# guanjq/targetdiff

Measured on NVIDIA H100. Metric: molecules/sec (1000-step sampling, CrossDocked pocket shape), higher is better.
Workload: dtype f32 (storage, LayerNorm, softmax, accumulation); GEMM operands as 2-piece bf16 splits on wgmma (3 products, ~16-bit operand mantissa)

## Files before the change

targetdiff_b200/csrc/edge_mlp_v4.cu:

```cuda
#include <stdio.h>
#include <stdlib.h>
#include <string.h>

#include "tdiff_common.cuh"
#include "hopper_mma.cuh"

namespace v4 {

constexpr int kTile = 64;
constexpr int kTabClassBytes = 2 * 128 * 128;
constexpr int kSrcStride = 512 + 32, kDst = 8;
constexpr int sSrc = 0, sDstRows = sSrc + kTile * kSrcStride, sMeta = sDstRows + kDst * 512, kStage = sMeta + kTile * 16;
constexpr int kMAtom = 32 * 128, kMPiece = 2 * kMAtom, kMImg = 2 * kMPiece;
template <int NOUT, bool FOLD>
struct Map {
  static constexpr int kCons = (NOUT == 128 && !FOLD) ? 3 : 2;
  static constexpr int kThreads = (kCons + 1) * 128;
  static constexpr int kProdRegs = kCons == 3 ? 32 : 40, kConsRegs = kCons == 3 ? 160 : 232;
  static constexpr int W = 0, T = W + 4 * 128 * 128, Par = T + kTabClassBytes, X = Par + 2 * 128 * 4,
                       M = X + kCons * 4 * 2 * 128 * 4, C = M + (FOLD ? kCons * kMImg : 0), Stage = C + (FOLD ? kCons * 32 * 4 : 0),
                       Bar = Stage + kCons * kStage, Smem = Bar + 8 * (1 + 2 * kCons);
  static constexpr bool kOrdered = kCons == 2;
  static constexpr int kPairBar = 1, kOrderBar = kPairBar + 2 * kCons, kFoldBar = kOrderBar + kCons;
  static_assert(M % 1024 == 0 && Stage % 128 == 0 && kStage % 128 == 0 && Smem <= 227 * 1024, "shared-memory map");
  static_assert(128 * kProdRegs + kCons * 128 * kConsRegs == kThreads * (65536 / kThreads / 8 * 8), "register split");
  static_assert(kFoldBar + kCons <= 16, "named barriers");
};

__device__ __forceinline__ uint32_t smem_u32(const void* p) { return (uint32_t)__cvta_generic_to_shared(p); }
__device__ __forceinline__ void mbar_init(uint32_t bar, uint32_t count) {
  asm volatile("mbarrier.init.shared::cta.b64 [%0], %1;" ::"r"(bar), "r"(count) : "memory");
}
__device__ __forceinline__ void mbar_wait(uint32_t bar, uint32_t parity) {
  asm volatile(
      "{\n\t.reg .pred p;\n\tWAIT_LOOP:\n\tmbarrier.try_wait.parity.shared::cta.b64 p, [%0], %1;\n\t@p bra WAIT_DONE;\n\tbra WAIT_LOOP;\n\t"
      "WAIT_DONE:\n\t}" ::"r"(bar), "r"(parity) : "memory");
}
__device__ __forceinline__ void mbar_expect_tx(uint32_t bar, uint32_t bytes) {
  asm volatile("mbarrier.arrive.expect_tx.shared::cta.b64 _, [%0], %1;" ::"r"(bar), "r"(bytes) : "memory");
}
__device__ __forceinline__ void bulk_g2s(uint32_t smem_dst, const void* gsrc, uint32_t bytes, uint32_t bar) {
  asm volatile("cp.async.bulk.shared::cluster.global.mbarrier::complete_tx::bytes [%0], [%1], %2, [%3];" ::"r"(smem_dst), "l"(gsrc), "r"(bytes),
               "r"(bar) : "memory");
}
__device__ __forceinline__ void fence_barrier_init() { asm volatile("fence.mbarrier_init.release.cluster;" ::: "memory"); }
__device__ __forceinline__ void mbar_arrive(uint32_t bar) { asm volatile("mbarrier.arrive.shared::cta.b64 _, [%0];" ::"r"(bar) : "memory"); }
__device__ __forceinline__ void mbar_expect_tx_only(uint32_t bar, uint32_t bytes) {
  asm volatile("mbarrier.expect_tx.shared::cta.b64 [%0], %1;" ::"r"(bar), "r"(bytes) : "memory");
}
__device__ __forceinline__ void named_bar_sync(int id, int nthreads) { asm volatile("bar.sync %0, %1;" ::"r"(id), "r"(nthreads) : "memory"); }
__device__ __forceinline__ void named_bar_arrive(int id, int nthreads) { asm volatile("bar.arrive %0, %1;" ::"r"(id), "r"(nthreads) : "memory"); }
template <int N> __device__ __forceinline__ void setmaxnreg_inc() { asm volatile("setmaxnreg.inc.sync.aligned.u32 %0;" ::"n"(N)); }
template <int N> __device__ __forceinline__ void setmaxnreg_dec() { asm volatile("setmaxnreg.dec.sync.aligned.u32 %0;" ::"n"(N)); }

__device__ __forceinline__ uint32_t cvt_bf16x2(float hi, float lo) {
  uint32_t d;
  asm("cvt.rn.bf16x2.f32 %0, %1, %2;" : "=r"(d) : "f"(hi), "f"(lo));
  return d;
}
__device__ __forceinline__ float ex2_approx(float x) { float y; asm("ex2.approx.ftz.f32 %0, %1;" : "=f"(y) : "f"(x)); return y; }
__device__ __forceinline__ void stg64(float* p, float a, float b) { asm volatile("st.global.v2.f32 [%0], {%1,%2};" ::"l"(p), "f"(a), "f"(b) : "memory"); }
__device__ __forceinline__ void stg128(float* p, float a, float b, float c, float d) {
  asm volatile("st.global.v4.f32 [%0], {%1,%2,%3,%4};" ::"l"(p), "f"(a), "f"(b), "f"(c), "f"(d) : "memory");
}

struct LnParams { float b[128]; float b2[128]; float mu[20]; };
struct AggArgs {
  const float* logits;
  const float* e_w;
  float* h;
  int key_softmax;
};

template <int N, int M, int LO_BIT>
__device__ __forceinline__ void transpose_reduce(float (&t)[N], int lane) {
  if constexpr (N > M) {
    constexpr int h = (N / M / 2) << LO_BIT;
    const bool up = lane & h;
#pragma unroll
    for (int i = 0; i < N / 2; ++i) {
      const float send = up ? t[i] : t[i + N / 2];
      const float keep = up ? t[i + N / 2] : t[i];
      t[i] = keep + __shfl_xor_sync(0xffffffffu, send, h);
    }
    transpose_reduce<N / 2, M, LO_BIT>(reinterpret_cast<float(&)[N / 2]>(t), lane);
  }
}
__device__ __forceinline__ void split2(float y0, float y1, uint32_t& hi, uint32_t& lo) {
  hi = cvt_bf16x2(y1, y0);
  const float r0 = __fsub_rn(y0, __uint_as_float(hi << 16)), r1 = __fsub_rn(y1, __uint_as_float(hi & 0xffff0000u));
  lo = cvt_bf16x2(r1, r0);
}

}

using namespace v4;

template <int NOUT, bool FOLD>
__global__ void __launch_bounds__(Map<NOUT, FOLD>::kThreads, 1)
edge_mlp_v4_kernel(const float* __restrict__ P, int zero_row, const int* __restrict__ src, const unsigned char* __restrict__ etype,
                   const float* __restrict__ dist_arr, const int* __restrict__ row_nodes, long long n_dst, long long split_dst,
                   const int* __restrict__ d_counts, int k, int offA, int offB, const unsigned char* __restrict__ w2_image,
                   const unsigned char* __restrict__ tab_image, float coeff, const float* __restrict__ qnode, float* __restrict__ out, int out_by_slot, AggArgs agg,
                   int cls, const __grid_constant__ LnParams lp) {
  static_assert(!FOLD || NOUT == 128, "the fold applies to the key MLPs");
  using L = Map<NOUT, FOLD>;
  constexpr int kCons = L::kCons, kThreads = L::kThreads;
  extern __shared__ __align__(1024) unsigned char smem_raw[];
  const uint32_t sbase = smem_u32(smem_raw);
  const uint32_t sW = sbase + L::W, sT = sbase + L::T, sBar = sbase + L::Bar;
  float* const s_b = reinterpret_cast<float*>(smem_raw + L::Par);
  float* const s_b2 = s_b + 128;
  const int tid = threadIdx.x, lane = tid & 31, warp = __shfl_sync(0xffffffffu, tid >> 5, 0);
  const int w = warp & 3, q = lane & 3;
  const int kshift = (k & (k - 1)) == 0 ? __ffs(k) - 1 : -1;
  auto row_dst = [&](long long idx, int& j) -> unsigned {
    const unsigned a = kshift >= 0 ? (unsigned)idx >> kshift : (unsigned)idx / (unsigned)k;
    j = (int)((unsigned)idx - a * (unsigned)k);
    return a;
  };

  if ((sbase & 1023u) != 0) __trap();
  if (d_counts) { n_dst = d_counts[0]; split_dst = d_counts[1]; }
  const long long n_rows = n_dst * k, split_rows = split_dst * k;
  const long long row_lo = cls ? split_rows : 0, row_hi = cls ? n_rows : split_rows;
  const long long n_tiles = row_hi > row_lo ? (row_hi - row_lo + kTile - 1) / kTile : 0;
  const long long my_tiles = (n_tiles > blockIdx.x) ? (n_tiles - blockIdx.x + gridDim.x - 1) / gridDim.x : 0;
  auto full_bar = [&](int c) { return sBar + 8u * (1 + c); };
  auto empty_bar = [&](int c) { return sBar + 8u * (1 + kCons + c); };

  constexpr int kWAtom = NOUT * 128;
  constexpr int kWPiece = 2 * kWAtom;
  constexpr uint32_t kWBytes = FOLD ? 4u * 128 * 128 : 2u * kWPiece;
  if (tid == 0) {
    mbar_init(sBar, 1);
    for (int c = 0; c < kCons; ++c) { mbar_init(full_bar(c), 32); mbar_init(empty_bar(c), 128); }
    fence_barrier_init();
    mbar_expect_tx(sBar, kWBytes + kTabClassBytes);
    bulk_g2s(sW, w2_image, kWBytes, sBar);
    bulk_g2s(sT, tab_image + (size_t)cls * kTabClassBytes, kTabClassBytes, sBar);
  }
  for (int i = tid; i < 128; i += kThreads) { s_b[i] = lp.b[i]; s_b2[i] = lp.b2[i]; }
  __syncthreads();

  if (warp < 4) {
    setmaxnreg_dec<L::kProdRegs>();
    if (warp >= kCons) return;
    const int c = warp;
    const uint32_t st = sbase + L::Stage + (uint32_t)c * kStage;
    for (long long it = c, use = 0; it < my_tiles; it += kCons, ++use) {
      const long long tile = blockIdx.x + it * (long long)gridDim.x, row0 = row_lo + tile * kTile;
      int j0;
      const unsigned a0 = row_dst(row0, j0);
      const long long last = (row0 + kTile - 1 < row_hi ? row0 + kTile - 1 : row_hi - 1);
      const int n_d = min(kDst, (int)(row_dst(last, j0) - a0) + 1);
      int s[2];
      int4 meta[2];
#pragma unroll
      for (int h = 0; h < 2; ++h) {
        const long long idx = row0 + lane + 32 * h;
        int jj = 0, ty = 3, slot = 0, node = -1;
        float dist = 0.f;
        s[h] = -1;
        if (idx < n_rows) {
          const unsigned a = row_dst(idx, jj);
          slot = a - a0 < (unsigned)kDst ? (int)(a - a0) + 1 : 0;
          node = row_nodes[a];
          if (node >= 0) {
            const size_t e = (size_t)node * k + jj;
            s[h] = src[e]; ty = etype[e]; dist = dist_arr[e];
          }
        }
        meta[h] = make_int4(node, s[h], __float_as_int(dist), ty | (slot << 8) | (jj << 16));
      }
      int dnode = -1;
      if (lane < n_d) dnode = row_nodes[a0 + lane];
      mbar_wait(empty_bar(c), (uint32_t)(use & 1) ^ 1u);
#pragma unroll
      for (int h = 0; h < 2; ++h) *reinterpret_cast<int4*>(smem_raw + L::Stage + c * kStage + sMeta + 16 * (lane + 32 * h)) = meta[h];
      if (lane == 0) mbar_expect_tx_only(full_bar(c), (uint32_t)(kTile + (FOLD ? 2 : 1) * n_d) * 512u);
      __syncwarp();
#pragma unroll
      for (int h = 0; h < 2; ++h)
        bulk_g2s(st + sSrc + (uint32_t)(lane + 32 * h) * kSrcStride, P + (size_t)(s[h] >= 0 ? s[h] : zero_row) * TD_NPROJ + offB, 512u, full_bar(c));
      if (lane < n_d) bulk_g2s(st + sDstRows + (uint32_t)lane * 512u, P + (size_t)(dnode >= 0 ? dnode : zero_row) * TD_NPROJ + offA, 512u, full_bar(c));
      if (FOLD && lane < n_d) bulk_g2s(st + sDstRows + (uint32_t)(2 + lane) * 512u, qnode + (size_t)(dnode >= 0 ? dnode : 0) * TD_H, 512u, full_bar(c));
      mbar_arrive(full_bar(c));
    }
    return;
  }

  setmaxnreg_inc<L::kConsRegs>();
  const int cwg = (warp >> 2) - 1;
  float mu[5];
#pragma unroll
  for (int m = 0; m < 5; ++m) mu[m] = lp.mu[5 * q + m];
  const float coeff2 = coeff * 1.4426950408889634f;
  mbar_wait(sBar, 0);

  const int r_base = 16 * w + (lane >> 2);
  const int pair_bar = L::kPairBar + 2 * cwg + (w >> 1);
  float* const xslot = reinterpret_cast<float*>(smem_raw + L::X) + (size_t)(cwg * 4 + w) * 256;
  float* const xpart = xslot + ((w & 1) ? -256 : 256);
  const bool do_agg = !FOLD && NOUT == 128 && qnode == nullptr && agg.logits != nullptr;
  const bool key_sm = NOUT == 128 && qnode != nullptr && agg.key_softmax;
  const unsigned char* const stage = smem_raw + L::Stage + cwg * kStage;
  const int ct = tid & 127, fu = ct & 7, fg = ct >> 3;
  const int fhd = 8 * (fg & 1) + 4 * (fu >> 2) + (fu & 3), fs = fu >> 2, frun = (fg >> 1) ^ (((fu >> 1) & 1) << 2);
  const int fn0 = 16 * ((fhd >> 1) & 1) + 2 * (fhd >> 2) + (fhd & 1);
  unsigned char* const mimg = smem_raw + L::M + cwg * kMImg;
  float* const s_c = reinterpret_cast<float*>(smem_raw + L::C) + cwg * 32;
  const int srow = k == 32 ? (w >> 1) : 0;
  const int order_mine = L::kOrderBar + cwg, order_next = L::kOrderBar + (cwg + 1) % kCons;
  auto order_wait = [&] { if constexpr (L::kOrdered) named_bar_sync(order_mine, 256); };
  auto order_pass = [&] { if constexpr (L::kOrdered) named_bar_arrive(order_next, 256); };
  const long long n_iter = (my_tiles + kCons - 1) / kCons;
  if (n_iter == 0) return;
  if (cwg == kCons - 1) order_pass();
  int set = 0;

  for (long long n = 0; n < n_iter; ++n, set ^= 1) {
    const long long it = n * kCons + cwg;
    if (it >= my_tiles) {
      if constexpr (L::kOrdered)
        for (int phase = 0; phase < 2; ++phase) { order_wait(); order_pass(); }
      continue;
    }
    const long long row0 = row_lo + (blockIdx.x + it * (long long)gridDim.x) * kTile;
    long long idx[2];
    int node[2], s[2], ty[2], jj[2], dsl[2];
    float dist[2];
    mbar_wait(full_bar(cwg), (uint32_t)(n & 1));
#pragma unroll
    for (int h = 0; h < 2; ++h) {
      idx[h] = row0 + r_base + 8 * h;
      const int4 m4 = *reinterpret_cast<const int4*>(stage + sMeta + 16 * (r_base + 8 * h));
      node[h] = m4.x; s[h] = m4.y; dist[h] = __int_as_float(m4.z);
      ty[h] = m4.w & 0xff; dsl[h] = ((m4.w >> 8) & 0xff) - 1; jj[h] = m4.w >> 16;
    }
    float ewp[2] = {0.f, 0.f};
    float4 qf[2][2];
    if constexpr (FOLD) {
#pragma unroll
      for (int h = 0; h < 2; ++h)
        if (key_sm && idx[h] < n_rows && node[h] >= 0) ewp[h] = agg.e_w[(size_t)node[h] * k + jj[h]];
#pragma unroll
      for (int sl = 0; sl < 2; ++sl)
#pragma unroll
        for (int hf = 0; hf < 2; ++hf) {
          float4 v = make_float4(0.f, 0.f, 0.f, 0.f);
          if (sl == 0 || k == 32) {
            v = *reinterpret_cast<const float4*>(stage + sDstRows + (2 + sl) * 512 + 32 * fhd + 16 * (hf ^ fs));
            v.x *= 0.35355339059327373f; v.y *= 0.35355339059327373f; v.z *= 0.35355339059327373f; v.w *= 0.35355339059327373f;
          }
          qf[sl][hf] = v;
        }
    }
    uint32_t ghi[4][4], glo[4][4];
#pragma unroll
    for (int h = 0; h < 2; ++h) {
      const bool ok = s[h] >= 0;
      float v[8];
#pragma unroll
      for (int m = 0; m < 5; ++m) {
        const float t = dist[h] - mu[m];
        v[m] = ok ? ex2_approx(coeff2 * (t * t)) : 0.0f;
      }
      v[5] = (ok && q == 3) ? 1.0f : 0.0f;
      v[6] = v[7] = 0.0f;
      const int half = ty[h] < 2 ? 1 : 0;
#pragma unroll
      for (int kk = 0; kk < 4; ++kk)
#pragma unroll
        for (int hk = 0; hk < 2; ++hk) {
          uint32_t hi, lo;
          split2(v[4 * (kk & 1) + 2 * hk], v[4 * (kk & 1) + 2 * hk + 1], hi, lo);
          const bool own = (kk >> 1) == half;
          ghi[kk][h + 2 * hk] = own ? hi : 0u;
          glo[kk][h + 2 * hk] = own ? lo : 0u;
        }
    }
    float x[64];
#pragma unroll
    for (int h = 0; h < 2; ++h) {
      const bool valid = s[h] >= 0;
      const float* ps = reinterpret_cast<const float*>(stage + sSrc + (r_base + 8 * h) * kSrcStride) + 2 * q;
      const float* pd = (dsl[h] >= 0 ? reinterpret_cast<const float*>(stage + sDstRows + dsl[h] * 512)
                                     : P + (size_t)(valid ? node[h] : zero_row) * TD_NPROJ + offA) + 2 * q;
#pragma unroll
      for (int i = 0; i < 16; ++i) {
        const float2 b = *reinterpret_cast<const float2*>(ps + 8 * i);
        float2 a = make_float2(0.f, 0.f);
        if (valid) a = *reinterpret_cast<const float2*>(pd + 8 * i);
        x[4 * i + 2 * h] = __fadd_rn(b.x, a.x);
        x[4 * i + 2 * h + 1] = __fadd_rn(b.y, a.y);
      }
    }
    mbar_arrive(empty_bar(cwg));
    wgmma_fence();
    order_wait();
#pragma unroll
    for (int term = 0; term < 3; ++term) {
#pragma unroll
      for (int kk = 0; kk < 4; ++kk)
        wgmma_n128_rs(x, term == 2 ? glo[kk] : ghi[kk], gmma_desc_sw128(sT + (term == 1 ? kTabClassBytes / 2 : 0) + kk * 32),
                      1u);
    }
    wgmma_commit();
    order_pass();
    if constexpr (FOLD) {
      const float* const w2s = reinterpret_cast<const float*>(smem_raw + L::W) + 8 * fhd;
#pragma unroll
      for (int jr = 0; jr < 2; ++jr) {
        const int f0 = 64 * jr + 8 * frun;
        float mv[2][8];
#pragma unroll
        for (int jf = 0; jf < 8; ++jf) {
          const float4 wa = *reinterpret_cast<const float4*>(w2s + (f0 + jf) * 128 + 4 * fs);
          const float4 wb = *reinterpret_cast<const float4*>(w2s + (f0 + jf) * 128 + 4 * (fs ^ 1));
#pragma unroll
          for (int sl = 0; sl < 2; ++sl) {
            const float4 qa = qf[sl][0], qb = qf[sl][1];
            const float pa = __fmaf_rn(wa.w, qa.w, __fmaf_rn(wa.z, qa.z, __fmaf_rn(wa.y, qa.y, wa.x * qa.x)));
            const float pb = __fmaf_rn(wb.w, qb.w, __fmaf_rn(wb.z, qb.z, __fmaf_rn(wb.y, qb.y, wb.x * qb.x)));
            mv[sl][jf] = pa + pb;
          }
        }
#pragma unroll
        for (int sl = 0; sl < 2; ++sl) {
          uint4 hi, lo;
          split2(mv[sl][0], mv[sl][1], hi.x, lo.x);
          split2(mv[sl][2], mv[sl][3], hi.y, lo.y);
          split2(mv[sl][4], mv[sl][5], hi.z, lo.z);
          split2(mv[sl][6], mv[sl][7], hi.w, lo.w);
          const int nr = fn0 + 8 * sl;
          const int off = jr * kMAtom + (nr >> 3) * 1024 + (nr & 7) * 128 + ((frun ^ (nr & 7)) << 4);
          *reinterpret_cast<uint4*>(mimg + off) = hi;
          *reinterpret_cast<uint4*>(mimg + kMPiece + off) = lo;
        }
      }
      if (fg < 2)
#pragma unroll
        for (int sl = 0; sl < 2; ++sl) {
          const float4 ba = *reinterpret_cast<const float4*>(s_b2 + 8 * fhd + 4 * fs), bb = *reinterpret_cast<const float4*>(s_b2 + 8 * fhd + 4 * (fs ^ 1));
          const float4 qa = qf[sl][0], qb = qf[sl][1];
          const float pa = __fmaf_rn(ba.w, qa.w, __fmaf_rn(ba.z, qa.z, __fmaf_rn(ba.y, qa.y, ba.x * qa.x)));
          const float pb = __fmaf_rn(bb.w, qb.w, __fmaf_rn(bb.z, qb.z, __fmaf_rn(bb.y, qb.y, bb.x * qb.x)));
          s_c[16 * sl + fhd] = pa + pb;
        }
      asm volatile("fence.proxy.async.shared::cta;" ::: "memory");
    }
    wgmma_wait_all();
    float rstd[2];
#pragma unroll
    for (int h = 0; h < 2; ++h) {
      float qa = 0.f, qb = 0.f;
#pragma unroll
      for (int i = 0; i < 16; ++i) {
        qa = __fmaf_rn(x[4 * i + 2 * h], x[4 * i + 2 * h], qa);
        qb = __fmaf_rn(x[4 * i + 2 * h + 1], x[4 * i + 2 * h + 1], qb);
      }
      float var = qa + qb;
      var += __shfl_xor_sync(0xffffffffu, var, 1);
      var += __shfl_xor_sync(0xffffffffu, var, 2);
      rstd[h] = rsqrtf(var * (1.0f / 128.0f) + 1e-5f);
    }
    uint32_t ahi[8][4], alo[8][4];
#pragma unroll
    for (int kk = 0; kk < 8; ++kk)
#pragma unroll
      for (int r = 0; r < 4; ++r) {
        const int h = r & 1, col = 16 * kk + 8 * (r >> 1) + 2 * q, e = 8 * kk + 2 * r;
        const float2 b = *reinterpret_cast<const float2*>(s_b + col);
        const float y0 = __fmaf_rn(x[e], rstd[h], b.x), y1 = __fmaf_rn(x[e + 1], rstd[h], b.y);
        split2(fmaxf(y0, 0.f), fmaxf(y1, 0.f), ahi[kk][r], alo[kk][r]);
      }
    float o[NOUT / 2];
    if constexpr (FOLD) {
      named_bar_sync(L::kFoldBar + cwg, 128);
#pragma unroll
      for (int sl = 0; sl < 2; ++sl) {
        const float4 cv = *reinterpret_cast<const float4*>(s_c + 16 * sl + 4 * q);
#pragma unroll
        for (int h = 0; h < 2; ++h) {
          o[4 * sl + 2 * h] = cv.x; o[4 * sl + 2 * h + 1] = cv.y;
          o[4 * (2 + sl) + 2 * h] = cv.z; o[4 * (2 + sl) + 2 * h + 1] = cv.w;
        }
      }
    }
    wgmma_fence();
    order_wait();
#pragma unroll
    for (int term = 0; term < 3; ++term) {
#pragma unroll
      for (int kk = 0; kk < 8; ++kk) {
        if constexpr (FOLD) {
          const uint64_t desc = gmma_desc_sw128(sbase + L::M + cwg * kMImg + (term == 1 ? kMPiece : 0) + (kk >> 2) * kMAtom + (kk & 3) * 32);
          wgmma_n32_rs(reinterpret_cast<float(&)[16]>(o), term == 2 ? alo[kk] : ahi[kk], desc, 1u);
        } else {
          const uint64_t desc = gmma_desc_sw128(sW + (term == 1 ? kWPiece : 0) + (kk >> 2) * kWAtom + (kk & 3) * 32);
          if constexpr (NOUT == 128) wgmma_n128_rs(o, term == 2 ? alo[kk] : ahi[kk], desc, (term | kk) ? 1u : 0u);
          else wgmma_n16_rs(o, term == 2 ? alo[kk] : ahi[kk], desc, (term | kk) ? 1u : 0u);
        }
      }
    }
    wgmma_commit();
    order_pass();
    wgmma_wait_all();

    long long orow[2];
    bool owrite[2];
#pragma unroll
    for (int h = 0; h < 2; ++h) {
      orow[h] = out_by_slot ? ((long long)node[h] * k + jj[h]) : idx[h];
      owrite[h] = idx[h] < n_rows && node[h] >= 0;
    }
    if constexpr (NOUT == 16) {
#pragma unroll
      for (int h = 0; h < 2; ++h)
        if (owrite[h])
#pragma unroll
          for (int i = 0; i < 2; ++i) {
            const float2 bb = *reinterpret_cast<const float2*>(s_b2 + 8 * i + 2 * q);
            stg64(out + (size_t)orow[h] * 16 + 8 * i + 2 * q, o[4 * i + 2 * h] + bb.x, o[4 * i + 2 * h + 1] + bb.y);
          }
    } else if (do_agg) {
      const int dnode = node[0];
      const bool active = dnode >= 0;
      const int ccol = 64 * (w & 1) + 2 * lane;
      float2 hin = make_float2(0.f, 0.f);
      if (active) hin = *reinterpret_cast<const float2*>(agg.h + (size_t)dnode * TD_H + ccol);
      float wt[2][16];
#pragma unroll
      for (int h = 0; h < 2; ++h)
#pragma unroll
        for (int i = 0; i < 4; ++i) {
          float4 t4 = make_float4(0.f, 0.f, 0.f, 0.f);
          if (active) t4 = __ldg(reinterpret_cast<const float4*>(agg.logits + (size_t)idx[h] * TD_HEADS + 4 * i));
          wt[h][4 * i] = t4.x; wt[h][4 * i + 1] = t4.y; wt[h][4 * i + 2] = t4.z; wt[h][4 * i + 3] = t4.w;
        }
      float t[32];
#pragma unroll
      for (int i = 0; i < 16; ++i) {
        const float2 bb = *reinterpret_cast<const float2*>(s_b2 + 8 * i + 2 * q);
#pragma unroll
        for (int c = 0; c < 2; ++c) {
          const float b = c ? bb.y : bb.x;
          t[2 * i + c] = __fadd_rn(__fmul_rn(__fadd_rn(o[4 * i + c], b), wt[0][i]), __fmul_rn(__fadd_rn(o[4 * i + 2 + c], b), wt[1][i]));
        }
      }
      transpose_reduce<32, 4, 2>(t, lane);
      float* slot = xslot + 128 * set;
      const int c0 = 16 * (lane >> 2) + 2 * q;
      *reinterpret_cast<float2*>(slot + c0) = make_float2(t[0], t[1]);
      *reinterpret_cast<float2*>(slot + c0 + 8) = make_float2(t[2], t[3]);
      named_bar_sync(pair_bar, 64);
      if (active) {
        const float* se = ((w & 1) ? xpart : xslot) + 128 * set;
        const float* so = ((w & 1) ? xslot : xpart) + 128 * set;
        const float2 a = *reinterpret_cast<const float2*>(se + ccol), b = *reinterpret_cast<const float2*>(so + ccol);
        *reinterpret_cast<float2*>(agg.h + (size_t)dnode * TD_H + ccol) = make_float2(hin.x + (a.x + b.x), hin.y + (a.y + b.y));
      }
    } else if (!FOLD && qnode == nullptr) {
#pragma unroll
      for (int h = 0; h < 2; ++h)
        if (owrite[h])
#pragma unroll
          for (int i = 0; i < 16; ++i) {
            const float2 bb = *reinterpret_cast<const float2*>(s_b2 + 8 * i + 2 * q);
            stg64(out + (size_t)orow[h] * 128 + 8 * i + 2 * q, o[4 * i + 2 * h] + bb.x, o[4 * i + 2 * h + 1] + bb.y);
          }
    } else {
      float lg[32];
      if constexpr (FOLD) {
#pragma unroll
        for (int h = 0; h < 2; ++h)
#pragma unroll
          for (int u = 0; u < 4; ++u) {
            const int e0 = 4 * (2 * (u >> 1)) + 2 * h + (u & 1);
            lg[4 * h + u] = srow ? o[e0 + 4] : o[e0];
          }
      } else {
#pragma unroll
        for (int h = 0; h < 2; ++h) {
          const float* qrow = qnode + (size_t)(node[h] >= 0 ? node[h] : 0) * TD_H + 2 * q;
#pragma unroll
          for (int i = 0; i < 16; ++i) {
            const float2 qv = __ldg(reinterpret_cast<const float2*>(qrow + 8 * i));
            const float2 bb = *reinterpret_cast<const float2*>(s_b2 + 8 * i + 2 * q);
            lg[8 * (i >> 2) + 4 * h + (i & 3)] = __fmaf_rn(o[4 * i + 2 * h + 1] + bb.y, qv.y, (o[4 * i + 2 * h] + bb.x) * qv.x);
          }
        }
        transpose_reduce<32, 8, 0>(lg, lane);
#pragma unroll
        for (int u = 0; u < 8; ++u) lg[u] *= 0.35355339059327373f;
      }
      if (key_sm) {
        bool valid_e[2];
        float ew[2];
#pragma unroll
        for (int h = 0; h < 2; ++h) {
          valid_e[h] = false; ew[h] = 0.f;
          if (owrite[h]) {
            valid_e[h] = s[h] >= 0;
            ew[h] = FOLD ? ewp[h] : agg.e_w[(size_t)node[h] * k + jj[h]];
          }
        }
        float mx[4], sm[4];
#pragma unroll
        for (int u = 0; u < 4; ++u) {
          lg[u] = valid_e[0] ? lg[u] * 1.4426950408889634f : -INFINITY;
          lg[4 + u] = valid_e[1] ? lg[4 + u] * 1.4426950408889634f : -INFINITY;
          mx[u] = fmaxf(lg[u], lg[4 + u]);
#pragma unroll
          for (int m = 4; m < 32; m <<= 1) mx[u] = fmaxf(mx[u], __shfl_xor_sync(0xffffffffu, mx[u], m));
        }
        if (lane < 4) *reinterpret_cast<float4*>(xslot + 4 * q) = make_float4(mx[0], mx[1], mx[2], mx[3]);
        named_bar_sync(pair_bar, 64);
        const float4 pm = *reinterpret_cast<const float4*>(xpart + 4 * q);
        mx[0] = fmaxf(mx[0], pm.x); mx[1] = fmaxf(mx[1], pm.y); mx[2] = fmaxf(mx[2], pm.z); mx[3] = fmaxf(mx[3], pm.w);
#pragma unroll
        for (int u = 0; u < 4; ++u) {
          lg[u] = valid_e[0] ? ex2_approx(lg[u] - mx[u]) : 0.0f;
          lg[4 + u] = valid_e[1] ? ex2_approx(lg[4 + u] - mx[u]) : 0.0f;
          sm[u] = lg[u] + lg[4 + u];
#pragma unroll
          for (int m = 4; m < 32; m <<= 1) sm[u] += __shfl_xor_sync(0xffffffffu, sm[u], m);
        }
        if (lane < 4) *reinterpret_cast<float4*>(xslot + 128 + 4 * q) = make_float4(sm[0], sm[1], sm[2], sm[3]);
        named_bar_sync(pair_bar, 64);
        const float4 ps = *reinterpret_cast<const float4*>(xpart + 128 + 4 * q);
        const float pl[4] = {ps.x, ps.y, ps.z, ps.w};
#pragma unroll
        for (int u = 0; u < 4; ++u) {
          const float l = sm[u] + pl[u];
          const float inv = l > 0.0f ? 1.0f / l : 0.0f;
          lg[u] = lg[u] * ew[0] * inv;
          lg[4 + u] = lg[4 + u] * ew[1] * inv;
        }
#pragma unroll
        for (int h = 0; h < 2; ++h)
          if (idx[h] < n_rows) stg128(out + (size_t)idx[h] * TD_HEADS + 4 * q, lg[4 * h], lg[4 * h + 1], lg[4 * h + 2], lg[4 * h + 3]);
      } else {
#pragma unroll
        for (int h = 0; h < 2; ++h)
          if (owrite[h]) stg128(out + (size_t)orow[h] * TD_HEADS + 4 * q, lg[4 * h], lg[4 * h + 1], lg[4 * h + 2], lg[4 * h + 3]);
      }
    }
  }
  if (cwg == 0) order_wait();
}

void td_launch_edge_mlp_v4(const float* P, int zero_row, const int* src, const unsigned char* etype, const float* dist, const int* row_nodes, long long n_dst,
                           long long split_dst, const int* d_counts, int k, const TdMlp& m, const float* h_offsets, float coeff,
                           const float* h_ln_b, const float* h_b2, const float* qnode, float* out, int out_by_slot,
                           const float* agg_logits, const float* agg_e_w, float* agg_h, int key_softmax, int sm_count, cudaStream_t st) {
  if (n_dst == 0) return;
  LnParams lp;
  memcpy(lp.b, h_ln_b, sizeof(lp.b));
  memset(lp.b2, 0, sizeof(lp.b2));
  memcpy(lp.b2, h_b2, sizeof(float) * (size_t)m.nout);
  memcpy(lp.mu, h_offsets, sizeof(lp.mu));
  static size_t opted128[TD_MAX_DEVICES] = {0}, opted16[TD_MAX_DEVICES] = {0}, optedF[TD_MAX_DEVICES] = {0};
  td_opt_in_smem(edge_mlp_v4_kernel<128, false>, Map<128, false>::Smem, opted128);
  td_opt_in_smem(edge_mlp_v4_kernel<16, false>, Map<16, false>::Smem, opted16);
  td_opt_in_smem(edge_mlp_v4_kernel<128, true>, Map<128, true>::Smem, optedF);
  AggArgs agg = {agg_logits, agg_e_w, agg_h, (key_softmax && k == 32) ? 1 : 0};
  const bool fold = m.nout == 128 && qnode && (k == 32 || k == 64);
  const long long n_cls[2] = {split_dst, n_dst - split_dst};
  for (int cls = 0; cls < 2; ++cls) {
    if (n_cls[cls] == 0) continue;
    const long long n_tiles = (n_cls[cls] * k + kTile - 1) / kTile;
    const int grid = (int)(n_tiles < sm_count ? n_tiles : sm_count);
    if (m.nout == 16)
      edge_mlp_v4_kernel<16, false><<<grid, Map<16, false>::kThreads, Map<16, false>::Smem, st>>>(
          P, zero_row, src, etype, dist, row_nodes, n_dst, split_dst, d_counts, k, m.offA, m.offB, m.w2_img, m.tabcls_img, coeff, nullptr,
          out, out_by_slot, agg, cls, lp);
    else if (fold)
      edge_mlp_v4_kernel<128, true><<<grid, Map<128, true>::kThreads, Map<128, true>::Smem, st>>>(
          P, zero_row, src, etype, dist, row_nodes, n_dst, split_dst, d_counts, k, m.offA, m.offB,
          reinterpret_cast<const unsigned char*>(m.w2t), m.tabcls_img, coeff, qnode, out, out_by_slot, agg, cls, lp);
    else
      edge_mlp_v4_kernel<128, false><<<grid, Map<128, false>::kThreads, Map<128, false>::Smem, st>>>(
          P, zero_row, src, etype, dist, row_nodes, n_dst, split_dst, d_counts, k, m.offA, m.offB, m.w2_img, m.tabcls_img, coeff, qnode,
          out, out_by_slot, agg, cls, lp);
  }
}
```

Measured before the change: 19.02.

## Replace key-MLP fold with TMA-staged query/h rows in a double-buffered epilogue area

Removes the FOLD variant, which precomputed W2·q images per tile on CUDA cores and ran a narrow N=32 wgmma. Key MLPs now use the plain 3-consumer N=128 path. The producer warp bulk-copies each destination node's query row (or h row for the value/aggregation role) and the edge weights into a double-buffered epilogue region guarded by new mbarriers, so epilogues read from shared memory instead of global. The trade-off is a full N=128 second GEMM for keys plus the qdot and transpose reduction, in exchange for removing the fold arithmetic and getting 3 consumers instead of 2.

```diff
diff --git a/targetdiff_b200/csrc/edge_mlp_v4.cu b/targetdiff_b200/csrc/edge_mlp_v4.cu
--- a/targetdiff_b200/csrc/edge_mlp_v4.cu
+++ b/targetdiff_b200/csrc/edge_mlp_v4.cu
@@ -1,6 +1,8 @@
 #include <stdio.h>
 #include <stdlib.h>
 #include <string.h>
+
+#include <type_traits>
 
 #include "tdiff_common.cuh"
 #include "hopper_mma.cuh"
@@ -11,20 +13,27 @@
 constexpr int kTabClassBytes = 2 * 128 * 128;
 constexpr int kSrcStride = 512 + 32, kDst = 8;
 constexpr int sSrc = 0, sDstRows = sSrc + kTile * kSrcStride, sMeta = sDstRows + kDst * 512, kStage = sMeta + kTile * 16;
-constexpr int kMAtom = 32 * 128, kMPiece = 2 * kMAtom, kMImg = 2 * kMPiece;
-template <int NOUT, bool FOLD>
+constexpr int sEpi = sDstRows + 2 * 512, kEpiHalf = 3 * 512, sEpiEw = 2 * 512;
+static_assert(sEpi + 2 * kEpiHalf == sMeta && sEpiEw + kTile * 4 <= kEpiHalf, "epilogue area");
+
+struct RoleKey {};
+struct RoleValue {};
+struct RolePlain {};
+
+template <int NOUT, class R>
 struct Map {
-  static constexpr int kCons = (NOUT == 128 && !FOLD) ? 3 : 2;
+  static constexpr bool kKey = std::is_same<R, RoleKey>::value, kValue = std::is_same<R, RoleValue>::value;
+  static_assert(NOUT == 128 || !(kKey || kValue), "the key and fused-aggregation epilogues need NOUT = 128");
+  static constexpr int kCons = NOUT == 128 ? 3 : 2;
   static constexpr int kThreads = (kCons + 1) * 128;
   static constexpr int kProdRegs = kCons == 3 ? 32 : 40, kConsRegs = kCons == 3 ? 160 : 232;
   static constexpr int W = 0, T = W + 4 * 128 * 128, Par = T + kTabClassBytes, X = Par + 2 * 128 * 4,
-                       M = X + kCons * 4 * 2 * 128 * 4, C = M + (FOLD ? kCons * kMImg : 0), Stage = C + (FOLD ? kCons * 32 * 4 : 0),
-                       Bar = Stage + kCons * kStage, Smem = Bar + 8 * (1 + 2 * kCons);
+                       Stage = X + kCons * 4 * 2 * 128 * 4, Bar = Stage + kCons * kStage, Smem = Bar + 8 * (1 + 4 * kCons);
   static constexpr bool kOrdered = kCons == 2;
-  static constexpr int kPairBar = 1, kOrderBar = kPairBar + 2 * kCons, kFoldBar = kOrderBar + kCons;
-  static_assert(M % 1024 == 0 && Stage % 128 == 0 && kStage % 128 == 0 && Smem <= 227 * 1024, "shared-memory map");
+  static constexpr int kPairBar = 1, kOrderBar = kPairBar + 2 * kCons;
+  static_assert(T % 1024 == 0 && Stage % 128 == 0 && kStage % 128 == 0 && Smem <= 227 * 1024, "shared-memory map");
   static_assert(128 * kProdRegs + kCons * 128 * kConsRegs == kThreads * (65536 / kThreads / 8 * 8), "register split");
-  static_assert(kFoldBar + kCons <= 16, "named barriers");
+  static_assert(kOrderBar + kCons <= 16, "named barriers");
 };
 
 __device__ __forceinline__ uint32_t smem_u32(const void* p) { return (uint32_t)__cvta_generic_to_shared(p); }
@@ -96,16 +105,16 @@
 
 using namespace v4;
 
-template <int NOUT, bool FOLD>
-__global__ void __launch_bounds__(Map<NOUT, FOLD>::kThreads, 1)
+template <int NOUT, class R>
+__global__ void __launch_bounds__(Map<NOUT, R>::kThreads, 1)
 edge_mlp_v4_kernel(const float* __restrict__ P, int zero_row, const int* __restrict__ src, const unsigned char* __restrict__ etype,
                    const float* __restrict__ dist_arr, const int* __restrict__ row_nodes, long long n_dst, long long split_dst,
                    const int* __restrict__ d_counts, int k, int offA, int offB, const unsigned char* __restrict__ w2_image,
                    const unsigned char* __restrict__ tab_image, float coeff, const float* __restrict__ qnode, float* __restrict__ out, int out_by_slot, AggArgs agg,
                    int cls, const __grid_constant__ LnParams lp) {
-  static_assert(!FOLD || NOUT == 128, "the fold applies to the key MLPs");
-  using L = Map<NOUT, FOLD>;
+  using L = Map<NOUT, R>;
   constexpr int kCons = L::kCons, kThreads = L::kThreads;
+  constexpr bool kKey = L::kKey, kValue = L::kValue;
   extern __shared__ __align__(1024) unsigned char smem_raw[];
   const uint32_t sbase = smem_u32(smem_raw);
   const uint32_t sW = sbase + L::W, sT = sbase + L::T, sBar = sbase + L::Bar;
@@ -126,15 +135,20 @@
   const long long row_lo = cls ? split_rows : 0, row_hi = cls ? n_rows : split_rows;
   const long long n_tiles = row_hi > row_lo ? (row_hi - row_lo + kTile - 1) / kTile : 0;
   const long long my_tiles = (n_tiles > blockIdx.x) ? (n_tiles - blockIdx.x + gridDim.x - 1) / gridDim.x : 0;
+  const bool epi = (kKey || kValue) && (k == 32 || k == 64);
+  const bool key_sm = kKey && agg.key_softmax && k == 32;
   auto full_bar = [&](int c) { return sBar + 8u * (1 + c); };
   auto empty_bar = [&](int c) { return sBar + 8u * (1 + kCons + c); };
+  auto epi_bar = [&](int c, int hf) { return sBar + 8u * (1 + 2 * kCons + 2 * c + hf); };
 
   constexpr int kWAtom = NOUT * 128;
   constexpr int kWPiece = 2 * kWAtom;
-  constexpr uint32_t kWBytes = FOLD ? 4u * 128 * 128 : 2u * kWPiece;
+  constexpr uint32_t kWBytes = 2u * kWPiece;
   if (tid == 0) {
     mbar_init(sBar, 1);
-    for (int c = 0; c < kCons; ++c) { mbar_init(full_bar(c), 32); mbar_init(empty_bar(c), 128); }
+    for (int c = 0; c < kCons; ++c) {
+      mbar_init(full_bar(c), 32); mbar_init(empty_bar(c), 128); mbar_init(epi_bar(c, 0), 128); mbar_init(epi_bar(c, 1), 128);
+    }
     fence_barrier_init();
     mbar_expect_tx(sBar, kWBytes + kTabClassBytes);
     bulk_g2s(sW, w2_image, kWBytes, sBar);
@@ -156,12 +170,14 @@
       const int n_d = min(kDst, (int)(row_dst(last, j0) - a0) + 1);
       int s[2];
       int4 meta[2];
+      float ew[2];
 #pragma unroll
       for (int h = 0; h < 2; ++h) {
         const long long idx = row0 + lane + 32 * h;
         int jj = 0, ty = 3, slot = 0, node = -1;
         float dist = 0.f;
         s[h] = -1;
+        ew[h] = 0.f;
         if (idx < n_rows) {
           const unsigned a = row_dst(idx, jj);
           slot = a - a0 < (unsigned)kDst ? (int)(a - a0) + 1 : 0;
@@ -169,22 +185,30 @@
           if (node >= 0) {
             const size_t e = (size_t)node * k + jj;
             s[h] = src[e]; ty = etype[e]; dist = dist_arr[e];
+            if (key_sm) ew[h] = agg.e_w[e];
           }
         }
         meta[h] = make_int4(node, s[h], __float_as_int(dist), ty | (slot << 8) | (jj << 16));
       }
       int dnode = -1;
       if (lane < n_d) dnode = row_nodes[a0 + lane];
+      const bool erow = epi && lane < n_d && dnode >= 0;
+      const int n_erow = __popc(__ballot_sync(0xffffffffu, erow));
+      const int ea = sEpi + (int)(use & 1) * kEpiHalf;
       mbar_wait(empty_bar(c), (uint32_t)(use & 1) ^ 1u);
-#pragma unroll
-      for (int h = 0; h < 2; ++h) *reinterpret_cast<int4*>(smem_raw + L::Stage + c * kStage + sMeta + 16 * (lane + 32 * h)) = meta[h];
-      if (lane == 0) mbar_expect_tx_only(full_bar(c), (uint32_t)(kTile + (FOLD ? 2 : 1) * n_d) * 512u);
+      if (epi) mbar_wait(epi_bar(c, (int)(use & 1)), (uint32_t)((use >> 1) & 1) ^ 1u);
+#pragma unroll
+      for (int h = 0; h < 2; ++h) {
+        *reinterpret_cast<int4*>(smem_raw + L::Stage + c * kStage + sMeta + 16 * (lane + 32 * h)) = meta[h];
+        if (key_sm) *reinterpret_cast<float*>(smem_raw + L::Stage + c * kStage + ea + sEpiEw + 4 * (lane + 32 * h)) = ew[h];
+      }
+      if (lane == 0) mbar_expect_tx_only(full_bar(c), (uint32_t)(kTile + n_d + n_erow) * 512u);
       __syncwarp();
 #pragma unroll
       for (int h = 0; h < 2; ++h)
         bulk_g2s(st + sSrc + (uint32_t)(lane + 32 * h) * kSrcStride, P + (size_t)(s[h] >= 0 ? s[h] : zero_row) * TD_NPROJ + offB, 512u, full_bar(c));
       if (lane < n_d) bulk_g2s(st + sDstRows + (uint32_t)lane * 512u, P + (size_t)(dnode >= 0 ? dnode : zero_row) * TD_NPROJ + offA, 512u, full_bar(c));
-      if (FOLD && lane < n_d) bulk_g2s(st + sDstRows + (uint32_t)(2 + lane) * 512u, qnode + (size_t)(dnode >= 0 ? dnode : 0) * TD_H, 512u, full_bar(c));
+      if (erow) bulk_g2s(st + (uint32_t)ea + (uint32_t)lane * 512u, (kKey ? qnode : agg.h) + (size_t)dnode * TD_H, 512u, full_bar(c));
       mbar_arrive(full_bar(c));
     }
     return;
@@ -202,14 +226,7 @@
   const int pair_bar = L::kPairBar + 2 * cwg + (w >> 1);
   float* const xslot = reinterpret_cast<float*>(smem_raw + L::X) + (size_t)(cwg * 4 + w) * 256;
   float* const xpart = xslot + ((w & 1) ? -256 : 256);
-  const bool do_agg = !FOLD && NOUT == 128 && qnode == nullptr && agg.logits != nullptr;
-  const bool key_sm = NOUT == 128 && qnode != nullptr && agg.key_softmax;
   const unsigned char* const stage = smem_raw + L::Stage + cwg * kStage;
-  const int ct = tid & 127, fu = ct & 7, fg = ct >> 3;
-  const int fhd = 8 * (fg & 1) + 4 * (fu >> 2) + (fu & 3), fs = fu >> 2, frun = (fg >> 1) ^ (((fu >> 1) & 1) << 2);
-  const int fn0 = 16 * ((fhd >> 1) & 1) + 2 * (fhd >> 2) + (fhd & 1);
-  unsigned char* const mimg = smem_raw + L::M + cwg * kMImg;
-  float* const s_c = reinterpret_cast<float*>(smem_raw + L::C) + cwg * 32;
   const int srow = k == 32 ? (w >> 1) : 0;
   const int order_mine = L::kOrderBar + cwg, order_next = L::kOrderBar + (cwg + 1) % kCons;
   auto order_wait = [&] { if constexpr (L::kOrdered) named_bar_sync(order_mine, 256); };
@@ -238,24 +255,6 @@
       node[h] = m4.x; s[h] = m4.y; dist[h] = __int_as_float(m4.z);
       ty[h] = m4.w & 0xff; dsl[h] = ((m4.w >> 8) & 0xff) - 1; jj[h] = m4.w >> 16;
     }
-    float ewp[2] = {0.f, 0.f};
-    float4 qf[2][2];
-    if constexpr (FOLD) {
-#pragma unroll
-      for (int h = 0; h < 2; ++h)
-        if (key_sm && idx[h] < n_rows && node[h] >= 0) ewp[h] = agg.e_w[(size_t)node[h] * k + jj[h]];
-#pragma unroll
-      for (int sl = 0; sl < 2; ++sl)
-#pragma unroll
-        for (int hf = 0; hf < 2; ++hf) {
-          float4 v = make_float4(0.f, 0.f, 0.f, 0.f);
-          if (sl == 0 || k == 32) {
-            v = *reinterpret_cast<const float4*>(stage + sDstRows + (2 + sl) * 512 + 32 * fhd + 16 * (hf ^ fs));
-            v.x *= 0.35355339059327373f; v.y *= 0.35355339059327373f; v.z *= 0.35355339059327373f; v.w *= 0.35355339059327373f;
-          }
-          qf[sl][hf] = v;
-        }
-    }
     uint32_t ghi[4][4], glo[4][4];
 #pragma unroll
     for (int h = 0; h < 2; ++h) {
@@ -308,48 +307,6 @@
     }
     wgmma_commit();
     order_pass();
-    if constexpr (FOLD) {
-      const float* const w2s = reinterpret_cast<const float*>(smem_raw + L::W) + 8 * fhd;
-#pragma unroll
-      for (int jr = 0; jr < 2; ++jr) {
-        const int f0 = 64 * jr + 8 * frun;
-        float mv[2][8];
-#pragma unroll
-        for (int jf = 0; jf < 8; ++jf) {
-          const float4 wa = *reinterpret_cast<const float4*>(w2s + (f0 + jf) * 128 + 4 * fs);
-          const float4 wb = *reinterpret_cast<const float4*>(w2s + (f0 + jf) * 128 + 4 * (fs ^ 1));
-#pragma unroll
-          for (int sl = 0; sl < 2; ++sl) {
-            const float4 qa = qf[sl][0], qb = qf[sl][1];
-            const float pa = __fmaf_rn(wa.w, qa.w, __fmaf_rn(wa.z, qa.z, __fmaf_rn(wa.y, qa.y, wa.x * qa.x)));
-            const float pb = __fmaf_rn(wb.w, qb.w, __fmaf_rn(wb.z, qb.z, __fmaf_rn(wb.y, qb.y, wb.x * qb.x)));
-            mv[sl][jf] = pa + pb;
-          }
-        }
-#pragma unroll
-        for (int sl = 0; sl < 2; ++sl) {
-          uint4 hi, lo;
-          split2(mv[sl][0], mv[sl][1], hi.x, lo.x);
-          split2(mv[sl][2], mv[sl][3], hi.y, lo.y);
-          split2(mv[sl][4], mv[sl][5], hi.z, lo.z);
-          split2(mv[sl][6], mv[sl][7], hi.w, lo.w);
-          const int nr = fn0 + 8 * sl;
-          const int off = jr * kMAtom + (nr >> 3) * 1024 + (nr & 7) * 128 + ((frun ^ (nr & 7)) << 4);
-          *reinterpret_cast<uint4*>(mimg + off) = hi;
-          *reinterpret_cast<uint4*>(mimg + kMPiece + off) = lo;
-        }
-      }
-      if (fg < 2)
-#pragma unroll
-        for (int sl = 0; sl < 2; ++sl) {
-          const float4 ba = *reinterpret_cast<const float4*>(s_b2 + 8 * fhd + 4 * fs), bb = *reinterpret_cast<const float4*>(s_b2 + 8 * fhd + 4 * (fs ^ 1));
-          const float4 qa = qf[sl][0], qb = qf[sl][1];
-          const float pa = __fmaf_rn(ba.w, qa.w, __fmaf_rn(ba.z, qa.z, __fmaf_rn(ba.y, qa.y, ba.x * qa.x)));
-          const float pb = __fmaf_rn(bb.w, qb.w, __fmaf_rn(bb.z, qb.z, __fmaf_rn(bb.y, qb.y, bb.x * qb.x)));
-          s_c[16 * sl + fhd] = pa + pb;
-        }
-      asm volatile("fence.proxy.async.shared::cta;" ::: "memory");
-    }
     wgmma_wait_all();
     float rstd[2];
 #pragma unroll
@@ -376,38 +333,22 @@
         split2(fmaxf(y0, 0.f), fmaxf(y1, 0.f), ahi[kk][r], alo[kk][r]);
       }
     float o[NOUT / 2];
-    if constexpr (FOLD) {
-      named_bar_sync(L::kFoldBar + cwg, 128);
-#pragma unroll
-      for (int sl = 0; sl < 2; ++sl) {
-        const float4 cv = *reinterpret_cast<const float4*>(s_c + 16 * sl + 4 * q);
-#pragma unroll
-        for (int h = 0; h < 2; ++h) {
-          o[4 * sl + 2 * h] = cv.x; o[4 * sl + 2 * h + 1] = cv.y;
-          o[4 * (2 + sl) + 2 * h] = cv.z; o[4 * (2 + sl) + 2 * h + 1] = cv.w;
-        }
-      }
-    }
     wgmma_fence();
     order_wait();
 #pragma unroll
     for (int term = 0; term < 3; ++term) {
 #pragma unroll
       for (int kk = 0; kk < 8; ++kk) {
-        if constexpr (FOLD) {
-          const uint64_t desc = gmma_desc_sw128(sbase + L::M + cwg * kMImg + (term == 1 ? kMPiece : 0) + (kk >> 2) * kMAtom + (kk & 3) * 32);
-          wgmma_n32_rs(reinterpret_cast<float(&)[16]>(o), term == 2 ? alo[kk] : ahi[kk], desc, 1u);
-        } else {
-          const uint64_t desc = gmma_desc_sw128(sW + (term == 1 ? kWPiece : 0) + (kk >> 2) * kWAtom + (kk & 3) * 32);
-          if constexpr (NOUT == 128) wgmma_n128_rs(o, term == 2 ? alo[kk] : ahi[kk], desc, (term | kk) ? 1u : 0u);
-          else wgmma_n16_rs(o, term == 2 ? alo[kk] : ahi[kk], desc, (term | kk) ? 1u : 0u);
-        }
+        const uint64_t desc = gmma_desc_sw128(sW + (term == 1 ? kWPiece : 0) + (kk >> 2) * kWAtom + (kk & 3) * 32);
+        if constexpr (NOUT == 128) wgmma_n128_rs(o, term == 2 ? alo[kk] : ahi[kk], desc, (term | kk) ? 1u : 0u);
+        else wgmma_n16_rs(o, term == 2 ? alo[kk] : ahi[kk], desc, (term | kk) ? 1u : 0u);
       }
     }
     wgmma_commit();
     order_pass();
     wgmma_wait_all();
 
+    const unsigned char* const earea = stage + sEpi + (int)(n & 1) * kEpiHalf;
     long long orow[2];
     bool owrite[2];
 #pragma unroll
@@ -424,12 +365,13 @@
             const float2 bb = *reinterpret_cast<const float2*>(s_b2 + 8 * i + 2 * q);
             stg64(out + (size_t)orow[h] * 16 + 8 * i + 2 * q, o[4 * i + 2 * h] + bb.x, o[4 * i + 2 * h + 1] + bb.y);
           }
-    } else if (do_agg) {
+    } else if constexpr (kValue) {
       const int dnode = node[0];
       const bool active = dnode >= 0;
       const int ccol = 64 * (w & 1) + 2 * lane;
       float2 hin = make_float2(0.f, 0.f);
-      if (active) hin = *reinterpret_cast<const float2*>(agg.h + (size_t)dnode * TD_H + ccol);
+      if (active)
+        hin = *reinterpret_cast<const float2*>(epi ? reinterpret_cast<const float*>(earea + 512 * srow) + ccol : agg.h + (size_t)dnode * TD_H + ccol);
       float wt[2][16];
 #pragma unroll
       for (int h = 0; h < 2; ++h)
@@ -461,7 +403,7 @@
         const float2 a = *reinterpret_cast<const float2*>(se + ccol), b = *reinterpret_cast<const float2*>(so + ccol);
         *reinterpret_cast<float2*>(agg.h + (size_t)dnode * TD_H + ccol) = make_float2(hin.x + (a.x + b.x), hin.y + (a.y + b.y));
       }
-    } else if (!FOLD && qnode == nullptr) {
+    } else if constexpr (!kKey) {
 #pragma unroll
       for (int h = 0; h < 2; ++h)
         if (owrite[h])
@@ -472,38 +414,37 @@
           }
     } else {
       float lg[32];
-      if constexpr (FOLD) {
+      auto logits = [&](auto q_at) {
 #pragma unroll
         for (int h = 0; h < 2; ++h)
 #pragma unroll
-          for (int u = 0; u < 4; ++u) {
-            const int e0 = 4 * (2 * (u >> 1)) + 2 * h + (u & 1);
-            lg[4 * h + u] = srow ? o[e0 + 4] : o[e0];
-          }
-      } else {
-#pragma unroll
-        for (int h = 0; h < 2; ++h) {
-          const float* qrow = qnode + (size_t)(node[h] >= 0 ? node[h] : 0) * TD_H + 2 * q;
-#pragma unroll
           for (int i = 0; i < 16; ++i) {
-            const float2 qv = __ldg(reinterpret_cast<const float2*>(qrow + 8 * i));
+            const float2 qv = q_at(h, i);
             const float2 bb = *reinterpret_cast<const float2*>(s_b2 + 8 * i + 2 * q);
             lg[8 * (i >> 2) + 4 * h + (i & 3)] = __fmaf_rn(o[4 * i + 2 * h + 1] + bb.y, qv.y, (o[4 * i + 2 * h] + bb.x) * qv.x);
           }
-        }
-        transpose_reduce<32, 8, 0>(lg, lane);
-#pragma unroll
-        for (int u = 0; u < 8; ++u) lg[u] *= 0.35355339059327373f;
-      }
+      };
+      if (epi) {
+        const float* const qs = reinterpret_cast<const float*>(earea + 512 * srow) + 2 * q;
+        logits([&](int, int i) { return *reinterpret_cast<const float2*>(qs + 8 * i); });
+      } else {
+        logits([&](int h, int i) {
+          return __ldg(reinterpret_cast<const float2*>(qnode + (size_t)(node[h] >= 0 ? node[h] : 0) * TD_H + 2 * q + 8 * i));
+        });
+      }
+      transpose_reduce<32, 8, 0>(lg, lane);
+#pragma unroll
+      for (int u = 0; u < 8; ++u) lg[u] *= 0.35355339059327373f;
       if (key_sm) {
         bool valid_e[2];
         float ew[2];
+        const float* const ews = reinterpret_cast<const float*>(earea + sEpiEw);
 #pragma unroll
         for (int h = 0; h < 2; ++h) {
           valid_e[h] = false; ew[h] = 0.f;
           if (owrite[h]) {
             valid_e[h] = s[h] >= 0;
-            ew[h] = FOLD ? ewp[h] : agg.e_w[(size_t)node[h] * k + jj[h]];
+            ew[h] = ews[r_base + 8 * h];
           }
         }
         float mx[4], sm[4];
@@ -547,6 +488,7 @@
           if (owrite[h]) stg128(out + (size_t)orow[h] * TD_HEADS + 4 * q, lg[4 * h], lg[4 * h + 1], lg[4 * h + 2], lg[4 * h + 3]);
       }
     }
+    if (epi) mbar_arrive(epi_bar(cwg, (int)(n & 1)));
   }
   if (cwg == 0) order_wait();
 }
@@ -561,28 +503,25 @@
   memset(lp.b2, 0, sizeof(lp.b2));
   memcpy(lp.b2, h_b2, sizeof(float) * (size_t)m.nout);
   memcpy(lp.mu, h_offsets, sizeof(lp.mu));
-  static size_t opted128[TD_MAX_DEVICES] = {0}, opted16[TD_MAX_DEVICES] = {0}, optedF[TD_MAX_DEVICES] = {0};
-  td_opt_in_smem(edge_mlp_v4_kernel<128, false>, Map<128, false>::Smem, opted128);
-  td_opt_in_smem(edge_mlp_v4_kernel<16, false>, Map<16, false>::Smem, opted16);
-  td_opt_in_smem(edge_mlp_v4_kernel<128, true>, Map<128, true>::Smem, optedF);
+  static size_t optedK[TD_MAX_DEVICES] = {0}, optedV[TD_MAX_DEVICES] = {0}, optedP[TD_MAX_DEVICES] = {0}, opted16[TD_MAX_DEVICES] = {0};
+  td_opt_in_smem(edge_mlp_v4_kernel<128, RoleKey>, Map<128, RoleKey>::Smem, optedK);
+  td_opt_in_smem(edge_mlp_v4_kernel<128, RoleValue>, Map<128, RoleValue>::Smem, optedV);
+  td_opt_in_smem(edge_mlp_v4_kernel<128, RolePlain>, Map<128, RolePlain>::Smem, optedP);
+  td_opt_in_smem(edge_mlp_v4_kernel<16, RolePlain>, Map<16, RolePlain>::Smem, opted16);
   AggArgs agg = {agg_logits, agg_e_w, agg_h, (key_softmax && k == 32) ? 1 : 0};
-  const bool fold = m.nout == 128 && qnode && (k == 32 || k == 64);
   const long long n_cls[2] = {split_dst, n_dst - split_dst};
   for (int cls = 0; cls < 2; ++cls) {
     if (n_cls[cls] == 0) continue;
     const long long n_tiles = (n_cls[cls] * k + kTile - 1) / kTile;
     const int grid = (int)(n_tiles < sm_count ? n_tiles : sm_count);
-    if (m.nout == 16)
-      edge_mlp_v4_kernel<16, false><<<grid, Map<16, false>::kThreads, Map<16, false>::Smem, st>>>(
-          P, zero_row, src, etype, dist, row_nodes, n_dst, split_dst, d_counts, k, m.offA, m.offB, m.w2_img, m.tabcls_img, coeff, nullptr,
-          out, out_by_slot, agg, cls, lp);
-    else if (fold)
-      edge_mlp_v4_kernel<128, true><<<grid, Map<128, true>::kThreads, Map<128, true>::Smem, st>>>(
-          P, zero_row, src, etype, dist, row_nodes, n_dst, split_dst, d_counts, k, m.offA, m.offB,
-          reinterpret_cast<const unsigned char*>(m.w2t), m.tabcls_img, coeff, qnode, out, out_by_slot, agg, cls, lp);
-    else
-      edge_mlp_v4_kernel<128, false><<<grid, Map<128, false>::kThreads, Map<128, false>::Smem, st>>>(
-          P, zero_row, src, etype, dist, row_nodes, n_dst, split_dst, d_counts, k, m.offA, m.offB, m.w2_img, m.tabcls_img, coeff, qnode,
-          out, out_by_slot, agg, cls, lp);
+    auto launch = [&](auto kernel, auto map, const float* qn) {
+      using L = decltype(map);
+      kernel<<<grid, L::kThreads, L::Smem, st>>>(P, zero_row, src, etype, dist, row_nodes, n_dst, split_dst, d_counts, k, m.offA, m.offB,
+                                                 m.w2_img, m.tabcls_img, coeff, qn, out, out_by_slot, agg, cls, lp);
+    };
+    if (m.nout == 16) launch(edge_mlp_v4_kernel<16, RolePlain>, Map<16, RolePlain>{}, nullptr);
+    else if (qnode) launch(edge_mlp_v4_kernel<128, RoleKey>, Map<128, RoleKey>{}, qnode);
+    else if (agg_logits) launch(edge_mlp_v4_kernel<128, RoleValue>, Map<128, RoleValue>{}, nullptr);
+    else launch(edge_mlp_v4_kernel<128, RolePlain>, Map<128, RolePlain>{}, nullptr);
   }
 }
```

Result: faster. 19.25 (median of 6 runs) (+1.2%).
